# JuliaMLTools/GraphNets.jl

Measured on AMD Instinct MI355X. Metric: edges updated/sec, GNBlock fwd, 1M-edge batch, higher is better.
Workload: dtype f32; 1 GPU; C2: one shared Erdos-Renyi graph, 100k nodes / 1M edges, batch_size=1 (BASELINE configs[1]); dims=(10, 5, 0)=>(3, 4, 5), edges_whole_job=1000000, edges_per_gpu=1000000, nodes_per_gpu=100000, graphs_per_gpu=1, parallelism=single GPU

## Files before the change

### graphnets.jl_amd/csrc/gnx_device.h

```cpp
#pragma once
#ifndef GNX_JIT
#include <hip/hip_runtime.h>
#endif

namespace gnx {

struct Tile {
  int n0, n1;
  int e0, e1;
  int g;
  int win0;
  int win1;
  int flags;
};

constexpr int kPdRowsCap = 28;

struct BlockArgs {
  int de, dn, dg;
  int oe, on, og;
  const float *We, *be, *Wn, *bn, *Wg, *bg;
  int act_e, act_n, act_g;
  const float *ef, *nf, *gf;
  float *ef_out, *nf_out, *gf_out;
// ... 13 lines not shown
  float ln_eps;
  int ln_mode;
  const float* ln_stats[3];
  int ln_inline_e;
  const int* packs;
  int n_packs;
  const float *ffe_w1, *ffe_b1, *ffe_w2, *ffe_b2, *ffe_g2, *ffe_be2;
  int ffe_act1, ffe_act2;
  void* ffe_scratch;
  const float* prev_partials;
  const float* prev_gf;
  float* prev_gf_out;
  int prev_blocks;
};

__device__ __forceinline__ float relu_f(float x) {
  float r;
  asm("v_max_f32 %0, 0, %1" : "=v"(r) : "v"(x));
  return r;
}

__device__ __forceinline__ float act_apply(float x, int act) {
  switch (act) {
    case 1: return relu_f(x);
    case 2: return tanhf(x);
    case 3: return 1.f / (1.f + expf(-x));
    case 4: return 0.5f * x * (1.f + tanhf(0.7978845608028654f * (x + 0.044715f * x * x * x)));
    default: return x;
  }
}
// ... 27 lines not shown
```

### graphnets.jl_amd/csrc/gnx_forward.hip

```cpp
#include <algorithm>
#include <cstdlib>

#include "gnx_launchers.h"
#include "gnx_step_hazard.h"

namespace gnx {

static_assert(GNX_ACT_IDENTITY == 0 && GNX_ACT_RELU == 1 && GNX_ACT_TANH == 2 && GNX_ACT_SIGMOID == 3 && GNX_ACT_GELU == 4,
              "act_apply (gnx_device.h) hard-codes the activation codes");

static int32_t check_block(const gnx_graphs* h, const gnx_block_params* p, int64_t R) {
  if (!h || !p) return fail(GNX_ERR_INVALID_ARG, "NULL handle or params");
  if (R <= 0) return fail(GNX_ERR_INVALID_ARG, "n_replicas must be >= 1");
  if (R > 1 && h->G != 1)
    return fail(GNX_ERR_INVALID_ARG, "n_replicas > 1 needs a single-graph handle (shared adjacency, batch.jl:66)");
  if (R > 65535) return fail(GNX_ERR_TOO_LARGE, "n_replicas exceeds the grid limit (65535)");
  const int d[6] = {p->de, p->dn, p->dg, p->oe, p->on, p->og};
  for (int i = 0; i < 6; ++i)
    if (d[i] < 0) return fail(GNX_ERR_DIMS, "negative feature width");
  if (p->de + p->dn + p->dg == 0) return fail(GNX_ERR_DIMS, "all input widths are 0 (gnblock.jl:48, batch.jl:56)");
  if (p->oe + p->on + p->og == 0) return fail(GNX_ERR_DIMS, "all output widths are 0 (gnblock.jl:49)");
  const gnx_dense* fn[3] = {&p->edgefn, &p->nodefn, &p->graphfn};
  const int out[3] = {p->oe, p->on, p->og};
  const int in[3] = {p->de + 2 * p->dn + p->dg, p->oe + p->dn + p->dg, p->oe + p->on + p->dg};
// ... 344 lines not shown

static StepSpans step_spans(const gnx_graphs* h, const gnx_block_params* p, int64_t R, const gnx_block_step& st, size_t elem, size_t ws_extent) {
  const void* const in[3] = {st.ef, st.nf, st.gf};
  const void* const out[3] = {st.ef_out, st.nf_out, st.gf_out};
  const long long rows[3] = {(long long)h->E, (long long)h->N, (long long)h->G};
  const int in_w[3] = {p->de, p->dn, p->dg}, out_w[3] = {p->oe, p->on, p->og};
  return step_spans_of(in, out, st.workspace, st.workspace_bytes, rows, in_w, out_w, R, elem, ws_extent);
}

static bool steps_overlap_applies(const gnx_graphs* h, const gnx_block_params* p, int64_t R, uint32_t flags, hipStream_t s) {
  if (!h || !p || matrix_core_widths(*p) || (flags & GNX_FLAG_FORCE_GENERIC) || form(GNX_FLAG_NO_FORK) || profile_enabled()) return false;
  if (check_block(h, p, R) != GNX_OK) return false;
  return block_narrow_takes(h, block_probe(h, p), s);
}

static int32_t steps_schedule(const gnx_graphs* h, const gnx_block_params* p, int32_t elem, const gnx_block_step* steps, int64_t n_steps, int64_t R,
                              uint32_t flags, void* stream, bool overlap) {
  const AuxHold hold = overlap ? take_aux(h, true) : AuxHold{};
  const gnx_graphs::AuxSet* aux = hold.set;
  hipStream_t str[2] = {(hipStream_t)stream, aux ? aux->stream : nullptr};
  gnx_pending_update pend[2]{};
  auto flush = [&](int k) -> int32_t {
    if (!pend[k].workspace) return GNX_OK;
    const int32_t rc = graph_update(h, p, elem, pend[k], R, flags, str[k]);
    pend[k] = gnx_pending_update{};
    return rc;
  };
  auto run = [&](const gnx_block_step& st, int k, gnx_pending_update* next) -> int32_t {
    const gnx_pending_update* prev = pend[k].workspace ? &pend[k] : nullptr;
    return chained_step(BlockCall{h, p, elem, st.ef, st.nf, st.gf, R, st.ef_out, st.nf_out, st.gf_out, st.workspace, st.workspace_bytes, flags, str[k], GNX_PHASE_ALL},
                        prev, next);
  };
  const bool bf16 = elem == GNX_ELEM_BF16;
  const bool valid = h && p && check_block(h, p, R) == GNX_OK;
  const size_t elem_bytes = bf16 ? 2 : sizeof(float);
  const size_t ws_extent = !valid ? 0 : bf16 ? typed_ws(h, p, R, true).total : block_ws(h, p, R).total;
  if (!aux) {
    StepSpans prev;
    for (int64_t i = 0; i < n_steps; ++i) {
      const gnx_block_step& st = steps[i];
      const StepSpans cur = valid ? step_spans(h, p, R, st, elem_bytes, ws_extent) : StepSpans{};
      if (pend[0].workspace && (pend[0].workspace == st.workspace || (p && p->og > 0 && pend[0].gf_out == st.gf_out) || steps_conflict(cur, prev))) {
        if (int32_t rc = flush(0)) return rc;
      }
      prev = cur;
      gnx_pending_update next{};
      if (int32_t rc = run(st, 0, &next)) {
        (void)flush(0);
        return rc;
      }
      pend[0] = next;
    }
    return flush(0);
  }
  GNX_HIP(hipEventRecord(aux->fork, str[0]));
  GNX_HIP(hipStreamWaitEvent(str[1], aux->fork, 0));
  StepSpans recent[3];
  int32_t rc = GNX_OK;
  for (int64_t i = 0; i < n_steps && rc == GNX_OK; ++i) {
    const gnx_block_step& st = steps[i];
    const int k = (int)(i & 1), o = k ^ 1;
    const StepSpans cur = step_spans(h, p, R, st, elem_bytes, ws_extent);
    const StepOrder ord = step_order(cur, recent, i);
    if (ord.flush_own && (rc = flush(k))) break;
    if (i >= 3) {
      const hipError_t e = hipStreamWaitEvent(str[k], aux->step[(i - 3) & 3], 0);
      if (e != hipSuccess) { rc = hip_fail(e, "gnx_block_forward_steps: ordering a step behind the step three before it"); break; }
    }
    if (ord.after_other) {
      if ((rc = flush(o))) break;
      hipEvent_t ev = o == 1 ? aux->join : aux->fork;
      hipError_t e = hipEventRecord(ev, str[o]);
      if (e == hipSuccess) e = hipStreamWaitEvent(str[k], ev, 0);
      if (e != hipSuccess) { rc = hip_fail(e, "gnx_block_forward_steps: ordering a step behind the other stream"); break; }
    }
    gnx_pending_update next{};
    rc = run(st, k, &next);
    if (rc != GNX_OK) break;
    pend[k] = next;
    if (const hipError_t e = hipEventRecord(aux->step[i & 3], str[k]); e != hipSuccess) { rc = hip_fail(e, "gnx_block_forward_steps: step event"); break; }
    recent[2] = recent[1]; recent[1] = recent[0]; recent[0] = cur;
  }
  const int32_t rf0 = flush(0), rf1 = flush(1);
  const hipError_t e1 = hipEventRecord(aux->join, str[1]);
  const hipError_t e2 = hipStreamWaitEvent(str[0], aux->join, 0);
  if (rc) return rc;
  if (rf0) return rf0;
  if (rf1) return rf1;
  GNX_HIP(e1);
  GNX_HIP(e2);
  return GNX_OK;
}

int32_t gnx_block_forward_steps(const gnx_graphs* h, const gnx_block_params* p, const gnx_block_step* steps, int64_t n_steps, int64_t R, uint32_t flags,
                                void* stream) {
  if (n_steps < 0 || (n_steps > 0 && !steps)) return fail(GNX_ERR_INVALID_ARG, "gnx_block_forward_steps: steps is NULL / n_steps is negative");
  if (flags & GNX_FLAG_DEFER_GRAPH_UPDATE) return fail(GNX_ERR_INVALID_ARG, "gnx_block_forward_steps finishes every step's graph update itself");
  DeviceTurn turn((hipStream_t)stream, p && matrix_core_widths(*p));
  FormScope forms(flags);
  return steps_schedule(h, p, GNX_ELEM_F32, steps, n_steps, R, flags, stream, n_steps > 1 && steps_overlap_applies(h, p, R, flags, (hipStream_t)stream));
// ... 334 lines not shown
```

### graphnets.jl_amd/csrc/gnx_launchers.h

```cpp
#pragma once
#include "gnx_internal.h"

namespace gnx {

struct EdgeLaunch {
  const Tile* tiles; size_t n_tiles; const float* ef; size_t E;
  struct { const float* stats; const float* g; const float* b; bool inline_stats; float eps; int mode; } ln;
  const float* We; int ldw;
  const float* psrc;
  const float* pdst;
  size_t N; const int* src; const int* dst; int act;
  float* out; float* colsum;
  float* agg_out; size_t n_agg_rows; const int* chunk_row0;
  int64_t R; void* scratch; hipStream_t stream;
};

int32_t launch_block_generic(const BlockArgs& a, int64_t R, int tile_n_cap, hipStream_t s, int phase);
int32_t launch_layernorm2(const float* x, size_t rows, int d, const gnx_layernorm& l1, const gnx_layernorm& l2, float eps, int eps_mode, float* y1, float* y2, hipStream_t s);
int32_t launch_ffn_residual(const float* z, const float* x, size_t rows, int d, const gnx_ffn& ff, float* out, hipStream_t s);
int32_t launch_pad(const gnx_graphs* h, int kind, bool pad, const float* src, int d, int64_t R, float* dst, hipStream_t s);
int32_t launch_calibration(int n, hipStream_t s);
int xent_blocks(int64_t cols);
int32_t launch_xent_backward(const float* logits, const float* targets, int d, int64_t cols, const float* upstream, float* dl, hipStream_t s);
int32_t launch_xent(const float* logits, const float* targets, int d, int64_t cols, float* out, float* ws, hipStream_t s);
int32_t launch_collapse(const gnx_graphs* h, const float* ef, int d, int64_t R, float* out, hipStream_t s);
int32_t launch_collapse_padded(const gnx_graphs* h, const float* ef, int d, int64_t R, float* out, hipStream_t s);
int32_t launch_fn_input(const gnx_graphs* h, int kind, const float* ef, int de, const float* nf, int dn, const float* gf, int dg, int64_t R, float* out, hipStream_t s);

int32_t launch_block_narrow(const gnx_graphs* h, const BlockArgs& a, int64_t R, hipStream_t s, int phase, bool bf16 = false);
void warm_block_narrow(const gnx_graphs* h, const gnx_block_params* p, bool bf16 = false);
bool block_narrow_ready(const gnx_graphs* h, const BlockArgs& a, hipStream_t s);
bool block_narrow_ffe_applies(const gnx_graphs* h, const BlockArgs& a, int act1, int act2);
bool block_narrow_chain_applies(const gnx_graphs* h, const BlockArgs& a, bool bf16 = false);
bool block_narrow_takes(const gnx_graphs* h, const BlockArgs& a, hipStream_t s, bool bf16 = false);
int32_t launch_block_narrow_chained(const gnx_graphs* h, const BlockArgs& a, int64_t R, hipStream_t s, bool bf16);
bool narrow_bf16_aot(const gnx_graphs* h, const BlockArgs& a);
int32_t launch_fused_bf16(const gnx_graphs* h, const BlockArgs& a, int64_t R, hipStream_t s, int phase);
int32_t launch_chained_bf16(const gnx_graphs* h, const BlockArgs& a, int64_t R, hipStream_t s);
bool jit_eligible(const BlockArgs& a, int ept);
int32_t jit_get(const BlockArgs& a, int ept, hipStream_t s, hipFunction_t* block, hipFunction_t* graph, bool bf16 = false);
int32_t jit_get_core_post3(int d0, int d1, int d2, hipStream_t s, hipFunction_t* fn);

bool core_narrow_width(int d);
int32_t launch_ln1_rows(const float* x, size_t rows, int d, const gnx_layernorm& l1, float eps, int eps_mode, float* y, hipStream_t s);
bool core_post3_applies(const size_t rows[3], const int d[3], const gnx_ffn ff[3], bool deferred, hipStream_t s);
int32_t launch_core_post3(const float* const x[3], const size_t rows[3], const int d[3], const gnx_layernorm l2[3], const gnx_ffn ff[3], float eps,
                          int eps_mode, float* const out[3], hipStream_t s, const BlockArgs* blk, int n_rows, bool skip_edges = false);
int32_t launch_core_post(const float* x, size_t rows, int d, const gnx_layernorm& l2, const gnx_ffn& ff, float eps, int eps_mode, float* out, hipStream_t s);

int32_t launch_block_wide(const gnx_graphs* h, const BlockArgs& a, int64_t R, hipStream_t s, int phase);
size_t wide_workspace_bytes(const gnx_graphs* h, const gnx_block_params* p, int64_t R);
void warm_block_wide(const gnx_graphs* h, const gnx_block_params* p, bool rows_gemm);
bool block_wide_ln_applies(const gnx_graphs* h, const BlockArgs& a);
// ... 69 lines not shown
```

### graphnets.jl_amd/csrc/gnx_narrow.hip

```cpp
#include <cstdlib>

#include "gnx_launchers.h"
#include "gnx_narrow_launch.h"
#include "gnx_wave_kernel.h"

namespace gnx {

#define GNX_NARROW_DIMS(X) \
  X(10, 5, 0, 3, 4)        \
  X(3, 4, 5, 3, 4)         \
  X(10, 5, 3, 3, 4)        \
  X(0, 2, 0, 2, 2)         \
  X(2, 2, 2, 2, 2)         \
  X(4, 3, 2, 3, 4)         \
  X(8, 8, 8, 16, 8)        \
  X(10, 5, 3, 10, 5)       \
  X(10, 5, 0, 10, 5)
static bool narrow_aot_listed(const BlockArgs& a) {
#define GNX_CASE(DE, DN, DG, OE, ON) \
  if (a.de == DE && a.dn == DN && a.dg == DG && a.oe == OE && a.on == ON) return true;
  GNX_NARROW_DIMS(GNX_CASE)
#undef GNX_CASE
  return false;
}
// ... 70 lines not shown
    const int32_t rc = launch_chained_bf16(h, a, R, s);
    return rc == 1 ? fail(GNX_ERR_INVALID_ARG, "internal: chained bf16 launch for a width set without that kernel") : rc;
  }
#define GNX_CASE(DE, DN, DG, OE, ON)                                                                                               \
  if (a.de == DE && a.dn == DN && a.dg == DG && a.oe == OE && a.on == ON) {                                                         \
    if constexpr (OE + ON > 0) {                                                                                                   \
      return h->G == 1 ? launch_wave_g<DE, DN, DG, OE, ON, 2, false, true, false, true>(h, a, R, s, 1)                              \
                       : launch_wave_g<DE, DN, DG, OE, ON, 2, false, false, false, true>(h, a, R, s, 1);                            \
    }                                                                                                                              \
  }
  GNX_NARROW_DIMS(GNX_CASE)
#undef GNX_CASE
  return fail(GNX_ERR_INVALID_ARG, "internal: chained launch for a width set without that kernel");
}

bool block_narrow_ffe_applies(const gnx_graphs* h, const BlockArgs& a, int act1, int act2) {
  return ln_aot(h, a) && a.ln_g[0] && act1 <= GNX_ACT_RELU && act2 <= GNX_ACT_RELU && a.act_e <= GNX_ACT_RELU && h->max_in_degree <= h->wtile_e_cap &&
         !form(GNX_FLAG_NO_FFE);
}

enum NarrowRoute { NR_NONE, NR_AOT, NR_JIT };
static NarrowRoute narrow_route(const gnx_graphs* h, const BlockArgs& a, hipStream_t s, bool bf16 = false) {
  if (a.n_wtiles == 0 || a.E == 0 || wants_ln(a)) return NR_NONE;
  auto jit_ok = [&]() {
    const int ept = jit_ept(h);
    hipFunction_t fb, fg;
    return ept && jit_get(a, ept, s, &fb, &fg, bf16) == GNX_OK;
  };
  static const bool jit_all = getenv("GNX_JIT_ALL") != nullptr;
  if (jit_all && jit_ok()) return NR_JIT;
// ... 37 lines not shown
```

### graphnets.jl_amd/csrc/gnx_narrow_bf16.hip

```cpp
#include "gnx_launchers.h"
#include "gnx_narrow_launch.h"
#include "gnx_wave_kernel.h"

namespace gnx {

#define GNX_NARROW_DIMS_BF16(X) \
  X(10, 5, 0, 3, 4)             \
  X(3, 4, 5, 3, 4)

bool narrow_bf16_aot(const gnx_graphs* h, const BlockArgs& a) {
#define GNX_CASE(DE, DN, DG, OE, ON)                                     \
  if (a.de == DE && a.dn == DN && a.dg == DG && a.oe == OE && a.on == ON) \
    return h->wtile_e_cap == 64 || h->wtile_e_cap == 128 || (h->wtile_e_cap == 256 && (DE + DN) * 4 <= 64);
  GNX_NARROW_DIMS_BF16(GNX_CASE)
#undef GNX_CASE
  return false;
}

int32_t launch_fused_bf16(const gnx_graphs* h, const BlockArgs& a, int64_t R, hipStream_t s, int phase) {
#define GNX_CASE(DE, DN, DG, OE, ON) \
  if (a.de == DE && a.dn == DN && a.dg == DG && a.oe == OE && a.on == ON) return launch_fused<DE, DN, DG, OE, ON, true>(h, a, R, s, phase);
  GNX_NARROW_DIMS_BF16(GNX_CASE)
#undef GNX_CASE
  return 1;
}

int32_t launch_chained_bf16(const gnx_graphs* h, const BlockArgs& a, int64_t R, hipStream_t s) {
#define GNX_CASE(DE, DN, DG, OE, ON)                                                                                               \
  if (a.de == DE && a.dn == DN && a.dg == DG && a.oe == OE && a.on == ON) {                                                         \
    if constexpr (OE + ON > 0) {                                                                                                   \
      return h->G == 1 ? launch_wave_g<DE, DN, DG, OE, ON, 2, false, true, false, true, true>(h, a, R, s, 1)                        \
                       : launch_wave_g<DE, DN, DG, OE, ON, 2, false, false, false, true, true>(h, a, R, s, 1);                      \
    }                                                                                                                              \
  }
  GNX_NARROW_DIMS_BF16(GNX_CASE)
#undef GNX_CASE
  return 1;
}

}
```

### graphnets.jl_amd/csrc/gnx_narrow_launch.h

```cpp
#pragma once
#include <cstdlib>

#include "gnx_device.h"
#include "gnx_wave_kernel.h"

namespace gnx {

static int partial_rows(const gnx_graphs* h) { return (int)(h->G == 1 ? (h->n_wtiles() + 3) / 4 : h->n_wtiles()); }

static int graph_update_threads(const gnx_graphs* h) {
  return graph_update_threads_for_rows(h->G == 1 ? (h->n_wtiles() + 3) / 4 : h->max_wtiles_per_graph);
}

template <int DE, int DN, int DG, int OE, int ON, int EPT, bool LN, bool ONEG, bool FFE = false, bool CHAIN = false, bool BF16 = false>
static int32_t launch_wave_g(const gnx_graphs* h, const BlockArgs& a, int64_t R, hipStream_t s, int phase) {
  constexpr int C = OE + ON;
  const int n_rows = partial_rows(h);
  const unsigned grid = (unsigned)((a.n_wtiles + 3) / 4) + (CHAIN ? (unsigned)a.prev_blocks : 0u);
  if (phase & 1) {
    ProfScope ps("k_block_wave", s);
#ifdef GNX_WAVE_STAMPS_BUILD
    static unsigned long long* d_dbg = nullptr;
    static size_t dbg_cap = 0;
    const char* dump = getenv("GNX_WAVE_STAMPS_DUMP");
// ... 15 lines not shown
    }
#endif
  }
  if ((phase & 2) && a.og > 0) {
    if constexpr (C > 0) {
      const int threads = graph_update_threads(h);
      const size_t lds = sizeof(float) * (size_t)graph_update_lds_floats(C, a.dg, a.og, threads);
      ProfScope ps("k_graph_t", s);
      GNX_LAUNCH((k_graph_t<C, ONEG, BF16>), dim3((unsigned)a.G, (unsigned)R), dim3(threads), lds, s, a, n_rows);
      GNX_HIP(hipGetLastError());
    }
  }
  return GNX_OK;
}

template <int DE, int DN, int DG, int OE, int ON, int EPT, bool BF16 = false>
static bool launch_wave_pack(const gnx_graphs* h, const BlockArgs& a, int64_t R, hipStream_t s, int phase, int32_t* rc) {
  constexpr int C = OE + ON;
  if constexpr (EPT != 2 || C == 0) return false;
  else {
    if (h->G <= 1 || h->n_packs <= 0 || !a.packs || phase != 3 || a.og <= 0 || form(GNX_FLAG_NO_PACK)) return false;
    ProfScope ps("k_block_wave", s);
    GNX_LAUNCH((k_block_wave<DE, DN, DG, OE, ON, EPT, false, false, true, false, false, BF16>), dim3((unsigned)h->n_packs, (unsigned)R), dim3(kPackThreads), 0, s, a, 0);
    const hipError_t e = hipGetLastError();
    *rc = e == hipSuccess ? GNX_OK : hip_fail(e, "k_block_wave<PACK>");
    return true;
  }
}

template <int DE, int DN, int DG, int OE, int ON, int EPT, bool LN = false, bool BF16 = false>
// ... 21 lines not shown
```

### graphnets.jl_amd/csrc/gnx_step_hazard.h

```cpp
#pragma once
#include <cstddef>
#include <cstdint>

namespace gnx {

struct ByteSpan {
  uintptr_t lo = 0, hi = 0;
};

inline ByteSpan byte_span(const void* p, size_t bytes) {
  ByteSpan s;
  if (p && bytes) { s.lo = reinterpret_cast<uintptr_t>(p); s.hi = s.lo + bytes; }
  return s;
}

inline bool spans_overlap(ByteSpan a, ByteSpan b) { return a.lo < a.hi && b.lo < b.hi && a.lo < b.hi && b.lo < a.hi; }

struct StepSpans {
  ByteSpan rd[3];
  ByteSpan wr[4];
};

inline StepSpans step_spans_of(const void* const in[3], const void* const out[3], const void* ws, size_t ws_bytes, const long long rows[3],
                               const int in_w[3], const int out_w[3], long long R, size_t elem, size_t ws_extent) {
// ... 16 lines not shown
    for (const ByteSpan& r : x.rd) if (spans_overlap(w, r)) return true;
  return false;
}

struct StepOrder {
  bool flush_own = false;
  bool after_other = false;
};
inline StepOrder step_order(const StepSpans& cur, const StepSpans* recent, long long i) {
  StepOrder o;
  o.flush_own = i >= 2 && steps_conflict(cur, recent[1]);
  o.after_other = (i >= 1 && steps_conflict(cur, recent[0])) || (i >= 3 && steps_conflict(cur, recent[2]));
  return o;
}

}
```

### graphnets.jl_amd/csrc/gnx_wave_kernel.h

```cpp
#pragma once
#include "gnx_device.h"

namespace gnx {

namespace {

constexpr int kThreads = 256;

struct __attribute__((packed, aligned(4))) F4u { float x, y, z, w; };
struct __attribute__((packed, aligned(4))) F3u { float x, y, z; };
struct __attribute__((packed, aligned(4))) F2u { float x, y; };

typedef const float __attribute__((address_space(4))) * cfloatp;
__device__ __forceinline__ cfloatp as_const(const float* p) { return reinterpret_cast<cfloatp>(reinterpret_cast<size_t>(p)); }

template <int D>
__device__ __forceinline__ void load_row(const float* __restrict__ p, float (&x)[D > 0 ? D : 1]) {
  constexpr int Q = D / 4, R = D % 4;
#pragma unroll
  for (int q = 0; q < Q; ++q) {
    const F4u v = *reinterpret_cast<const F4u*>(p + 4 * q);
    x[4 * q] = v.x; x[4 * q + 1] = v.y; x[4 * q + 2] = v.z; x[4 * q + 3] = v.w;
  }
  if constexpr (R == 3) {
// ... 619 lines not shown
#define GNX_WSTAMP(i) do { } while (0)
#endif
constexpr int kPackThreads = 512;
typedef const BlockArgs __attribute__((address_space(4))) * cargsp;
template <bool FRESH>
__device__ __forceinline__ auto phase_args(const BlockArgs& a) {
  if constexpr (FRESH) {
    cargsp p = (cargsp)__builtin_amdgcn_kernarg_segment_ptr();
    asm volatile("" : "+s"(p));
    return p;
  } else {
    return &a;
  }
}

template <int DE, int DN, int DG, int OE, int ON, int EPT, bool LN, bool ONEG, bool PACK, bool FFE, bool CHAIN, bool BF16 = false>
__device__ __forceinline__ void block_wave_body(BlockArgs& a, int n_rows) {
  static_assert(!(PACK && ONEG), "packs are for batches of several graphs");
  static_assert(!BF16 || (!FFE && !LN), "bf16 features: the plain block forward and its chained form");
  static_assert(!CHAIN || (!PACK && !FFE && !LN && OE + ON > 0), "CHAIN: the two-launch form of a plain block");
  static_assert(!FFE || (LN && DE == OE && DE > 0 && EPT == 2 && (DE + DN) * OE > 96 && ((DE + DN) * OE) % 2 == 0 && GNX_WAVE_PK && !PACK),
                "FFE: a core's block (dims => dims) with LayerNorm on load, two edges per lane, streamed weights");
  constexpr int OE1 = OE > 0 ? OE : 1, ON1 = ON > 0 ? ON : 1, DE1 = DE > 0 ? DE : 1, DN1 = DN > 0 ? DN : 1, DG1 = DG > 0 ? DG : 1;
  constexpr int TEW = 64 * EPT;
  constexpr int C = OE + ON, C1 = C > 0 ? C : 1;
  constexpr int WAVES = (PACK ? kPackThreads : kThreads) / 64;
  constexpr int WSL = wave_slice_floats(OE, EPT);
  constexpr bool FRESH = FFE || (CHAIN && BF16 && !ONEG);
  __shared__ __attribute__((aligned(16))) float s_mem[WAVES * WSL];

  const int lane = threadIdx.x & 63;
  const int wv = __builtin_amdgcn_readfirstlane(threadIdx.x >> 6);
// ... 46 lines not shown
  float* s_out = s_mem + wv * WSL;
  float* s_pd = s_out + (TEW * OE + 4);
  unsigned char* s_dst = reinterpret_cast<unsigned char*>(s_pd + (64 * OE + 4));

  const cintp tw = reinterpret_cast<cintp>(reinterpret_cast<size_t>(A0->wtiles)) + (size_t)wt * (sizeof(Tile) / sizeof(int));
  const int n0 = tw[0], n1 = tw[1], e0 = tw[2], e1 = tw[3], g = tw[4];
  if constexpr (PACK) {
    tile_g = g; tile_cnt = tw[7];
    const cintp pk = reinterpret_cast<cintp>(reinterpret_cast<size_t>(A0->packs)) + (size_t)xcd_tile(bx, gx) * WAVES;
    const int wprev = wv > 0 ? pk[wv > 0 ? wv - 1 : 0] : -1;
    owner = wprev < 0 || (reinterpret_cast<cintp>(reinterpret_cast<size_t>(A0->wtiles)) + (size_t)wprev * (sizeof(Tile) / sizeof(int)))[4] != g;
  }
  const int nn = n1 - n0, ne = e1 - e0;
  GNX_WSTAMP(1);

  const size_t r = blockIdx.y;
  const auto* __restrict__ ef = DE > 0 ? feat<BF16>(A0->ef) + r * (size_t)A0->E * DE : nullptr;
  const auto* __restrict__ nf = DN > 0 ? feat<BF16>(A0->nf) + r * (size_t)A0->N * DN : nullptr;
  const cfloatp gf = DG > 0 && !BF16 ? as_const(A0->gf + (r * (size_t)A0->G + g) * DG) : nullptr;

  const bool is_node = lane < nn;
  const int nl = lane < nn ? lane : nn - 1;
  const int cp0 = A0->colptr[n0 + nl], cp1 = A0->colptr[n0 + nl + 1];
  float xn[1][DN1];
  if constexpr (DN > 0) load_row<DN>(nf + (size_t)(n0 + nl) * DN, xn[0]);
  const int cn0 = ne < TEW ? ne : TEW;
  float x[EPT][DE1];
  float xs[EPT][DN1];
  int src[EPT];
#pragma unroll
  for (int i = 0; i < EPT; ++i) {
    int ec = lane + 64 * i;
    ec = ec < cn0 ? ec : cn0 - 1;
    int e = e0 + (ec > 0 ? ec : 0);
    e = e < A0->E ? e : A0->E - 1;
    if constexpr (DE > 0) load_row<DE>(ef + (size_t)e * DE, x[i]);
    if constexpr (DN > 0) src[i] = A0->rowval[e];
  }
  if constexpr (DN > 0) {
#pragma unroll
    for (int i = 0; i < EPT; ++i) load_row<DN>(nf + (size_t)src[i] * DN, xs[i]);
  }
  float gfr[1][DG1];
  if constexpr (BF16) {
    if constexpr (DG > 0) load_row<DG>(feat<true>(A0->gf) + (r * (size_t)A0->G + g) * DG, gfr[0]);
  } else {
#pragma unroll
    for (int k = 0; k < DG; ++k) gfr[0][k] = gf[k];
  }
  if constexpr (LN) {
    ln_row<DN>(xn[0], A0->ln_g[1], A0->ln_b[1], A0->ln_eps, A0->ln_mode);
    ln_row<DG>(gfr[0], A0->ln_g[2], A0->ln_b[2], A0->ln_eps, A0->ln_mode);
  }
  GNX_WSTAMP(2);
  const auto A1 = phase_args<FRESH>(a);
  const cfloatp We = as_const(A1->We);
  const cfloatp be = as_const(A1->be ? A1->be : k_zero_bias);
  if (is_node) {
    if (nn > 1)
      for (int e = cp0 - e0; e < cp1 - e0; ++e) s_dst[e] = (unsigned char)lane;
    if constexpr (OE > 0) {
      float b[1][OE1];
#pragma unroll
      for (int j = 0; j < OE; ++j) b[0][j] = be[j];
      fma_rows<DG, OE, 1, DG1>(We + (DE + 2 * DN) * OE, gfr, b);
      fma_rows<DN, OE, 1, DN1>(We + (DE + DN) * OE, xn, b);
#pragma unroll
      for (int j = 0; j < OE; ++j) s_pd[lane * OE + j] = b[0][j];
    }
  }
  __builtin_amdgcn_wave_barrier();
  GNX_WSTAMP(3);
// ... 87 lines not shown
        fma_rows<DE, OE, EPT, DE1>(We, x, acc);
        fma_rows<DN, OE, EPT, DN1>(We + DE * OE, xs, acc);
      }
#pragma unroll
      for (int i = 0; i < EPT; ++i) {
        const int el = lane + 64 * i;
        if constexpr (FFE) {
          if (A1->act_e == 1) {
#pragma unroll
            for (int j = 0; j < OE; ++j) acc[i][j] = relu_f(acc[i][j]);
          }
        } else {
          act_row<OE1>(acc[i], A1->act_e);
        }
        if (valid[i]) {
          if constexpr (!FFE) store_row<OE>(feat<BF16>(A1->ef_out) + (r * (size_t)A1->E + e0 + c0 + el) * OE, acc[i]);
          if (nn > 1 || FFE) {
#pragma unroll
            for (int j = 0; j < OE; ++j) s_out[el * OE + j] = acc[i][j];
          }
          if (nn == 1) {
#pragma unroll
            for (int j = 0; j < OE; ++j) psum[j] += acc[i][j];
          }
        }
      }
      if constexpr (FFE) {
#pragma unroll
        for (int m = 0; m < EPT; ++m) ffv[m] = valid[m];
        ff_row0 = r * (size_t)A1->E + e0 + c0 + lane;
      }
// ... 4 lines not shown
        const int el = lane + 64 * i;
        if (el < cn) {
          const int dl = nn > 1 ? (int)s_dst[el] : 0;
          float acc[OE1];
#pragma unroll
          for (int j = 0; j < OE; ++j) acc[j] = s_pd[dl * OE + j];
#pragma unroll
          for (int k = 0; k < DE; ++k)
#pragma unroll
            for (int j = 0; j < OE; ++j) acc[j] = fmaf(We[k * OE + j], x[i][k], acc[j]);
#pragma unroll
          for (int k = 0; k < DN; ++k)
#pragma unroll
            for (int j = 0; j < OE; ++j) acc[j] = fmaf(We[(DE + k) * OE + j], xs[i][k], acc[j]);
          act_row<OE1>(acc, A1->act_e);
          store_row<OE>(feat<BF16>(A1->ef_out) + (r * (size_t)A1->E + e0 + c0 + el) * OE, acc);
          if (nn > 1) {
#pragma unroll
            for (int j = 0; j < OE; ++j) s_out[el * OE + j] = acc[j];
          } else {
#pragma unroll
            for (int j = 0; j < OE; ++j) psum[j] += acc[j];
          }
        }
      }
    }
    if constexpr (FFE) break;
  }
  __builtin_amdgcn_wave_barrier();
  GNX_WSTAMP(4);
  const auto A2 = phase_args<FRESH>(a);
  const cfloatp Wn = as_const(A2->Wn);
  const cfloatp bn = as_const(A2->bn ? A2->bn : k_zero_bias);

  float v[C1];
#pragma unroll
  for (int c = 0; c < C1; ++c) v[c] = 0.f;
  if constexpr (OE > 0) {
    if (nn == 1) {
#pragma unroll
      for (int j = 0; j < OE; ++j) {
        const float tot = wave_sum(psum[j]);
        v[j] = lane == 0 ? tot : 0.f;
      }
    } else if (is_node) {
      for (int e = cp0 - e0; e < cp1 - e0; ++e) {
#pragma unroll
        for (int j = 0; j < OE; ++j) v[j] += s_out[e * OE + j];
// ... 3 lines not shown
  if constexpr (ON > 0) {
    if (is_node) {
      float acc1[1][ON1];
      float (&acc)[ON1] = acc1[0];
#pragma unroll
      for (int j = 0; j < ON; ++j) acc[j] = bn[j];
      fma_rows<DG, ON, 1, DG1>(Wn + (OE + DN) * ON, gfr, acc1);
      float vin[1][OE1];
#pragma unroll
      for (int k = 0; k < OE; ++k) vin[0][k] = v[k];
      fma_rows<OE, ON, 1, OE1>(Wn, vin, acc1);
      fma_rows<DN, ON, 1, DN1>(Wn + OE * ON, xn, acc1);
      act_row<ON1>(acc, A2->act_n);
#pragma unroll
      for (int j = 0; j < ON; ++j) v[OE + j] = acc[j];
      store_row<ON>(feat<BF16>(A2->nf_out) + (r * (size_t)A2->N + n0 + lane) * ON, acc);
    }
  }

  if (A2->og > 0) {
    if constexpr (C > 0) {
      float sel[(C + 15) / 16];
#pragma unroll
      for (int g = 0; g < (C + 15) / 16; ++g) sel[g] = 0.f;
#pragma unroll
      for (int c = 0; c < C; ++c) {
        const float s16 = row16_sum(v[c]);
        sel[c >> 4] = (lane & 15) == (c & 15) ? s16 : sel[c >> 4];
      }
      float tot = 0.f;
#pragma unroll
// ... 7 lines not shown
    }
  }
  GNX_WSTAMP(5);
  } while (0);
#ifdef GNX_WAVE_STAMPS_BUILD
  if (active && g_wave_dbg && lane == 0 && blockIdx.y == 0) {
    wst_[6] = clock64();
    unsigned long long* o = g_wave_dbg + (size_t)wt * 8;
    for (int i = 0; i < 7; ++i) o[i] = wst_[i];
    o[7] = ((unsigned long long)__builtin_amdgcn_s_getreg((31 << 11) | 20) << 32) | __builtin_amdgcn_s_getreg((31 << 11) | 4);
  }
#endif
  const auto A3 = phase_args<FRESH>(a);
  if (A3->og > 0) {
    if constexpr (C > 0) {
      const size_t r = blockIdx.y;
      constexpr int CP = (C + 3) / 4 * 4;
      float* __restrict__ pbase = A3->partials + r * (size_t)n_rows * CP;
      if constexpr (PACK) {
        __shared__ float s_rows[WAVES][C1];
        if (lane < C) s_rows[wv][lane] = active ? mine : 0.f;
        GraphWaveRegs gr;
        if (active && owner) graph_wave_prefetch<C>(a, lane, gr);
        __syncthreads();
        if (active && owner) {
          float rr[8];
#pragma unroll
          for (int k = 0; k < 8; ++k) rr[k] = (k < tile_cnt && wv + k < WAVES && lane < C) ? 0.f + s_rows[(wv + k) < WAVES ? wv + k : 0][lane < C ? lane : 0] : 0.f;
          const float xs = ((rr[0] + rr[1]) + (rr[2] + rr[3])) + ((rr[4] + rr[5]) + (rr[6] + rr[7]));
          graph_update_wave<C, BF16>(a, xs, tile_g, r, lane, s_mem + wv * WSL, gr);
        }
      } else if constexpr (ONEG) {
        __shared__ float s_blk[WAVES][C1];
// ... 54 lines not shown
    }
  }
}

template <int DE, int DN, int DG, int OE, int ON, int EPT, bool LN = false, bool ONEG = false, bool PACK = false, bool FFE = false, bool CHAIN = false,
          bool BF16 = false>
__global__ __launch_bounds__(PACK ? kPackThreads : kThreads) __attribute__((amdgpu_num_sgpr(GNX_WAVE_SGPRS))) void k_block_wave(BlockArgs a, int n_rows) {
  static_assert(!FFE, "the FFE form is k_block_wave_ffe");
  block_wave_body<DE, DN, DG, OE, ON, EPT, LN, ONEG, PACK, false, CHAIN, BF16>(a, n_rows);
}
template <int DE, int DN, int DG, int OE, int ON, int EPT, bool ONEG>
__global__ __launch_bounds__(kThreads) __attribute__((amdgpu_waves_per_eu(4))) void k_block_wave_ffe(BlockArgs a, int n_rows) {
  block_wave_body<DE, DN, DG, OE, ON, EPT, true, ONEG, false, true, false>(a, n_rows);
}

template <int C, bool ONEG = false, bool BF16 = false>
__global__ void k_graph_t(BlockArgs a, int n_rows) {
  extern __shared__ float s_g[];
  constexpr int CP = (C + 3) / 4 * 4;
  const int g = blockIdx.x;
  const int t0 = ONEG ? 0 : a.wtile_off[g], t1 = ONEG ? (a.n_wtiles + 3) / 4 : a.wtile_off[g + 1];
  const float* base = a.partials + blockIdx.y * (size_t)n_rows * CP;
  if (blockDim.x == 64) graph_update_rows<C, true, 16, BF16>(a, a.gf, a.gf_out, base, g, blockIdx.y, t0, t1, (int)threadIdx.x, 64, s_g);
  else graph_update_rows<C, false, 16, BF16>(a, a.gf, a.gf_out, base, g, blockIdx.y, t0, t1, (int)threadIdx.x, (int)blockDim.x, s_g);
}

}
```

Baseline: 54.16 billion edges/s.

## Batch independent forward steps into one multi-slot kernel launch

Groups up to eight consecutive non-conflicting block-forward steps into a single launch. Each step's input and output pointers go into a table placed after BlockArgs in the kernel arguments, and grid.y selects the step's slot. This is meant to cut per-step launch and event overhead and let several steps fill the GPU together. In exchange it adds more hazard-grouping logic and larger kernel arguments, and it only applies to single-replica narrow width sets.

```diff
diff --git a/graphnets.jl_amd/csrc/gnx_device.h b/graphnets.jl_amd/csrc/gnx_device.h
--- a/graphnets.jl_amd/csrc/gnx_device.h
+++ b/graphnets.jl_amd/csrc/gnx_device.h
@@ -51,6 +51,17 @@
   int prev_blocks;
 };
 
+struct RunSlot {
+  const float *ef, *nf, *gf;
+  float *ef_out, *nf_out, *gf_out;
+  float* partials;
+};
+constexpr int kRunSlots = 8;
+struct RunTable {
+  RunSlot slot[kRunSlots];
+};
+constexpr unsigned kRunTableOffset = (unsigned)((sizeof(BlockArgs) + 7) / 8 * 8);
+
 __device__ __forceinline__ float relu_f(float x) {
   float r;
   asm("v_max_f32 %0, 0, %1" : "=v"(r) : "v"(x));
diff --git a/graphnets.jl_amd/csrc/gnx_forward.hip b/graphnets.jl_amd/csrc/gnx_forward.hip
--- a/graphnets.jl_amd/csrc/gnx_forward.hip
+++ b/graphnets.jl_amd/csrc/gnx_forward.hip
@@ -382,10 +382,22 @@
   return block_narrow_takes(h, block_probe(h, p), s);
 }
 
+constexpr int kStepsRunDefault = 8;
+static_assert(kRunMax == kRunSlots, "gnx_step_hazard.h groups what gnx_device.h's table holds");
+static int steps_run_max() {
+  static const int v = [] {
+    const char* e = getenv("GNX_STEPS_RUN_MAX");
+    const int n = e && *e ? atoi(e) : kStepsRunDefault;
+    return n < 1 ? 1 : (n > kRunMax ? kRunMax : n);
+  }();
+  return v;
+}
+
 static int32_t steps_schedule(const gnx_graphs* h, const gnx_block_params* p, int32_t elem, const gnx_block_step* steps, int64_t n_steps, int64_t R,
                               uint32_t flags, void* stream, bool overlap) {
   const AuxHold hold = overlap ? take_aux(h, true) : AuxHold{};
   const gnx_graphs::AuxSet* aux = hold.set;
+  const bool two = aux != nullptr;
   hipStream_t str[2] = {(hipStream_t)stream, aux ? aux->stream : nullptr};
   gnx_pending_update pend[2]{};
   auto flush = [&](int k) -> int32_t {
@@ -403,36 +415,52 @@
   const bool valid = h && p && check_block(h, p, R) == GNX_OK;
   const size_t elem_bytes = bf16 ? 2 : sizeof(float);
   const size_t ws_extent = !valid ? 0 : bf16 ? typed_ws(h, p, R, true).total : block_ws(h, p, R).total;
-  if (!aux) {
-    StepSpans prev;
-    for (int64_t i = 0; i < n_steps; ++i) {
-      const gnx_block_step& st = steps[i];
-      const StepSpans cur = valid ? step_spans(h, p, R, st, elem_bytes, ws_extent) : StepSpans{};
-      if (pend[0].workspace && (pend[0].workspace == st.workspace || (p && p->og > 0 && pend[0].gf_out == st.gf_out) || steps_conflict(cur, prev))) {
-        if (int32_t rc = flush(0)) return rc;
+  bool can_fuse = valid && R == 1 && !(flags & GNX_FLAG_FORCE_GENERIC) && steps_run_max() > 1 && !profile_enabled();
+  auto slot_of = [&](const gnx_block_step& st, RunSlot& sl, BlockArgs* run_args) -> bool {
+    Prepared q(BlockCall{h, p, elem, st.ef, st.nf, st.gf, R, st.ef_out, st.nf_out, st.gf_out, st.workspace, st.workspace_bytes, flags, str[0], GNX_PHASE_ALL});
+    if (q.rc) return false;
+    if (run_args) {
+      if (!block_narrow_run_applies(h, q.a, bf16)) return can_fuse = false;
+      *run_args = q.a;
+    }
+    sl = RunSlot{q.a.ef, q.a.nf, q.a.gf, q.a.ef_out, q.a.nf_out, q.a.gf_out, q.a.partials};
+    return true;
+  };
+  if (two) {
+    GNX_HIP(hipEventRecord(aux->fork, str[0]));
+    GNX_HIP(hipStreamWaitEvent(str[1], aux->fork, 0));
+  }
+  RunSpans recent[3];
+  int32_t rc = GNX_OK;
+  int64_t i = 0;
+  for (int64_t j = 0; i < n_steps && rc == GNX_OK; ++j) {
+    const gnx_block_step& st = steps[i];
+    RunSpans cur;
+    RunTable tab{};
+    BlockArgs run_args{};
+    cur.step[0] = valid ? step_spans(h, p, R, st, elem_bytes, ws_extent) : StepSpans{};
+    cur.n = 1;
+    if (can_fuse && n_steps - i >= 2) {
+      RunSpans win = cur;
+      while (i + win.n < n_steps) {
+        const StepSpans sp = step_spans(h, p, R, steps[i + win.n], elem_bytes, ws_extent);
+        if (!run_takes(win, sp, steps_run_max())) break;
+        win.step[win.n++] = sp;
       }
-      prev = cur;
-      gnx_pending_update next{};
-      if (int32_t rc = run(st, 0, &next)) {
-        (void)flush(0);
-        return rc;
-      }
-      pend[0] = next;
-    }
-    return flush(0);
-  }
-  GNX_HIP(hipEventRecord(aux->fork, str[0]));
-  GNX_HIP(hipStreamWaitEvent(str[1], aux->fork, 0));
-  StepSpans recent[3];
-  int32_t rc = GNX_OK;
-  for (int64_t i = 0; i < n_steps && rc == GNX_OK; ++i) {
-    const gnx_block_step& st = steps[i];
-    const int k = (int)(i & 1), o = k ^ 1;
-    const StepSpans cur = step_spans(h, p, R, st, elem_bytes, ws_extent);
-    const StepOrder ord = step_order(cur, recent, i);
-    if (ord.flush_own && (rc = flush(k))) break;
-    if (i >= 3) {
-      const hipError_t e = hipStreamWaitEvent(str[k], aux->step[(i - 3) & 3], 0);
+      bool ok = window_is_run(win.n, i, n_steps, steps_run_max());
+      for (int z = 0; ok && z < win.n; ++z) ok = slot_of(steps[i + z], tab.slot[z], z == 0 ? &run_args : nullptr);
+      if (ok) cur = win;
+    }
+    const int k = two ? (int)(j & 1) : 0, o = k ^ 1;
+    StepOrder ord;
+    if (two) {
+      ord = run_order(cur, recent, j);
+    } else {
+      ord.flush_own = pend[0].workspace && (pend[0].workspace == st.workspace || (p && p->og > 0 && pend[0].gf_out == st.gf_out) || runs_conflict(cur, recent[0]));
+    }
+    if ((ord.flush_own || cur.n > 1) && (rc = flush(k))) break;
+    if (two && j >= 3) {
+      const hipError_t e = hipStreamWaitEvent(str[k], aux->step[(j - 3) & 3], 0);
       if (e != hipSuccess) { rc = hip_fail(e, "gnx_block_forward_steps: ordering a step behind the step three before it"); break; }
     }
     if (ord.after_other) {
@@ -442,16 +470,26 @@
       if (e == hipSuccess) e = hipStreamWaitEvent(str[k], ev, 0);
       if (e != hipSuccess) { rc = hip_fail(e, "gnx_block_forward_steps: ordering a step behind the other stream"); break; }
     }
-    gnx_pending_update next{};
-    rc = run(st, k, &next);
+    if (cur.n > 1) {
+      rc = launch_block_narrow_run(h, run_args, tab, cur.n, str[k], bf16);
+    } else {
+      gnx_pending_update next{};
+      rc = run(st, k, &next);
+      if (rc == GNX_OK) pend[k] = next;
+    }
     if (rc != GNX_OK) break;
-    pend[k] = next;
-    if (const hipError_t e = hipEventRecord(aux->step[i & 3], str[k]); e != hipSuccess) { rc = hip_fail(e, "gnx_block_forward_steps: step event"); break; }
+    if (two) {
+      if (const hipError_t e = hipEventRecord(aux->step[j & 3], str[k]); e != hipSuccess) { rc = hip_fail(e, "gnx_block_forward_steps: step event"); break; }
+    }
     recent[2] = recent[1]; recent[1] = recent[0]; recent[0] = cur;
-  }
-  const int32_t rf0 = flush(0), rf1 = flush(1);
-  const hipError_t e1 = hipEventRecord(aux->join, str[1]);
-  const hipError_t e2 = hipStreamWaitEvent(str[0], aux->join, 0);
+    i += cur.n;
+  }
+  const int32_t rf0 = flush(0), rf1 = two ? flush(1) : GNX_OK;
+  hipError_t e1 = hipSuccess, e2 = hipSuccess;
+  if (two) {
+    e1 = hipEventRecord(aux->join, str[1]);
+    e2 = hipStreamWaitEvent(str[0], aux->join, 0);
+  }
   if (rc) return rc;
   if (rf0) return rf0;
   if (rf1) return rf1;
diff --git a/graphnets.jl_amd/csrc/gnx_launchers.h b/graphnets.jl_amd/csrc/gnx_launchers.h
--- a/graphnets.jl_amd/csrc/gnx_launchers.h
+++ b/graphnets.jl_amd/csrc/gnx_launchers.h
@@ -37,6 +37,10 @@
 bool narrow_bf16_aot(const gnx_graphs* h, const BlockArgs& a);
 int32_t launch_fused_bf16(const gnx_graphs* h, const BlockArgs& a, int64_t R, hipStream_t s, int phase);
 int32_t launch_chained_bf16(const gnx_graphs* h, const BlockArgs& a, int64_t R, hipStream_t s);
+bool block_narrow_run_applies(const gnx_graphs* h, const BlockArgs& a, bool bf16);
+bool narrow_bf16_run(const gnx_graphs* h, const BlockArgs& a);
+int32_t launch_block_narrow_run(const gnx_graphs* h, const BlockArgs& a, const RunTable& t, int Z, hipStream_t s, bool bf16);
+int32_t launch_run_bf16(const gnx_graphs* h, const BlockArgs& a, const RunTable& t, int Z, hipStream_t s);
 bool jit_eligible(const BlockArgs& a, int ept);
 int32_t jit_get(const BlockArgs& a, int ept, hipStream_t s, hipFunction_t* block, hipFunction_t* graph, bool bf16 = false);
 int32_t jit_get_core_post3(int d0, int d1, int d2, hipStream_t s, hipFunction_t* fn);
diff --git a/graphnets.jl_amd/csrc/gnx_narrow.hip b/graphnets.jl_amd/csrc/gnx_narrow.hip
--- a/graphnets.jl_amd/csrc/gnx_narrow.hip
+++ b/graphnets.jl_amd/csrc/gnx_narrow.hip
@@ -108,6 +108,38 @@
   return fail(GNX_ERR_INVALID_ARG, "internal: chained launch for a width set without that kernel");
 }
 
+#define GNX_NARROW_RUN_DIMS(X) \
+  X(10, 5, 0, 3, 4)            \
+  X(3, 4, 5, 3, 4)             \
+  X(10, 5, 3, 3, 4)            \
+  X(0, 2, 0, 2, 2)             \
+  X(2, 2, 2, 2, 2)             \
+  X(4, 3, 2, 3, 4)
+bool block_narrow_run_applies(const gnx_graphs* h, const BlockArgs& a, bool bf16) {
+  if (!block_narrow_chain_applies(h, a, bf16)) return false;
+  if (bf16) return narrow_bf16_run(h, a);
+#define GNX_CASE(DE, DN, DG, OE, ON) \
+  if (a.de == DE && a.dn == DN && a.dg == DG && a.oe == OE && a.on == ON) return true;
+  GNX_NARROW_RUN_DIMS(GNX_CASE)
+#undef GNX_CASE
+  return false;
+}
+int32_t launch_block_narrow_run(const gnx_graphs* h, const BlockArgs& a, const RunTable& t, int Z, hipStream_t s, bool bf16) {
+  if (bf16) {
+    const int32_t rc = launch_run_bf16(h, a, t, Z, s);
+    return rc == 1 ? fail(GNX_ERR_INVALID_ARG, "internal: bf16 run launch for a width set without that kernel") : rc;
+  }
+#define GNX_CASE(DE, DN, DG, OE, ON)                                                                                               \
+  if (a.de == DE && a.dn == DN && a.dg == DG && a.oe == OE && a.on == ON) {                                                         \
+    if constexpr (OE + ON > 0) {                                                                                                   \
+      return h->G == 1 ? launch_wave_run<DE, DN, DG, OE, ON, true>(h, a, t, Z, s) : launch_wave_run<DE, DN, DG, OE, ON, false>(h, a, t, Z, s); \
+    }                                                                                                                              \
+  }
+  GNX_NARROW_RUN_DIMS(GNX_CASE)
+#undef GNX_CASE
+  return fail(GNX_ERR_INVALID_ARG, "internal: run launch for a width set without that kernel");
+}
+
 bool block_narrow_ffe_applies(const gnx_graphs* h, const BlockArgs& a, int act1, int act2) {
   return ln_aot(h, a) && a.ln_g[0] && act1 <= GNX_ACT_RELU && act2 <= GNX_ACT_RELU && a.act_e <= GNX_ACT_RELU && h->max_in_degree <= h->wtile_e_cap &&
          !form(GNX_FLAG_NO_FFE);
diff --git a/graphnets.jl_amd/csrc/gnx_narrow_bf16.hip b/graphnets.jl_amd/csrc/gnx_narrow_bf16.hip
--- a/graphnets.jl_amd/csrc/gnx_narrow_bf16.hip
+++ b/graphnets.jl_amd/csrc/gnx_narrow_bf16.hip
@@ -38,4 +38,25 @@
   return 1;
 }
 
+#define GNX_NARROW_RUN_DIMS_BF16(X) \
+  X(10, 5, 0, 3, 4, false)          \
+  X(3, 4, 5, 3, 4, true)
+bool narrow_bf16_run(const gnx_graphs* h, const BlockArgs& a) {
+#define GNX_CASE(DE, DN, DG, OE, ON, SEVERAL) \
+  if (a.de == DE && a.dn == DN && a.dg == DG && a.oe == OE && a.on == ON) return h->G == 1 || SEVERAL;
+  GNX_NARROW_RUN_DIMS_BF16(GNX_CASE)
+#undef GNX_CASE
+  return false;
 }
+int32_t launch_run_bf16(const gnx_graphs* h, const BlockArgs& a, const RunTable& t, int Z, hipStream_t s) {
+#define GNX_CASE(DE, DN, DG, OE, ON, SEVERAL)                                                                \
+  if (a.de == DE && a.dn == DN && a.dg == DG && a.oe == OE && a.on == ON) {                                   \
+    if (h->G == 1) return launch_wave_run<DE, DN, DG, OE, ON, true, true>(h, a, t, Z, s);                     \
+    if constexpr (SEVERAL) return launch_wave_run<DE, DN, DG, OE, ON, false, true>(h, a, t, Z, s);            \
+  }
+  GNX_NARROW_RUN_DIMS_BF16(GNX_CASE)
+#undef GNX_CASE
+  return 1;
+}
+
+}
diff --git a/graphnets.jl_amd/csrc/gnx_narrow_launch.h b/graphnets.jl_amd/csrc/gnx_narrow_launch.h
--- a/graphnets.jl_amd/csrc/gnx_narrow_launch.h
+++ b/graphnets.jl_amd/csrc/gnx_narrow_launch.h
@@ -53,6 +53,26 @@
   return GNX_OK;
 }
 
+template <int DE, int DN, int DG, int OE, int ON, bool ONEG, bool BF16 = false>
+static int32_t launch_wave_run(const gnx_graphs* h, const BlockArgs& a, const RunTable& t, int Z, hipStream_t s) {
+  constexpr int C = OE + ON;
+  if (Z < 1 || Z > kRunSlots) return fail(GNX_ERR_INVALID_ARG, "internal: a run of more steps than the table has slots");
+  const int n_rows = partial_rows(h);
+  {
+    ProfScope ps("k_block_wave", s);
+    GNX_LAUNCH((k_block_wave_run<DE, DN, DG, OE, ON, 2, ONEG, BF16>), dim3((unsigned)((a.n_wtiles + 3) / 4), (unsigned)Z), dim3(kThreads), 0, s, a, t, n_rows);
+    GNX_HIP(hipGetLastError());
+  }
+  if (a.og > 0) {
+    const int threads = graph_update_threads(h);
+    const size_t lds = sizeof(float) * (size_t)graph_update_lds_floats(C, a.dg, a.og, threads);
+    ProfScope ps("k_graph_t", s);
+    GNX_LAUNCH((k_graph_run<C, ONEG, BF16>), dim3((unsigned)a.G, (unsigned)Z), dim3(threads), lds, s, a, t, n_rows);
+    GNX_HIP(hipGetLastError());
+  }
+  return GNX_OK;
+}
+
 template <int DE, int DN, int DG, int OE, int ON, int EPT, bool BF16 = false>
 static bool launch_wave_pack(const gnx_graphs* h, const BlockArgs& a, int64_t R, hipStream_t s, int phase, int32_t* rc) {
   constexpr int C = OE + ON;
diff --git a/graphnets.jl_amd/csrc/gnx_step_hazard.h b/graphnets.jl_amd/csrc/gnx_step_hazard.h
--- a/graphnets.jl_amd/csrc/gnx_step_hazard.h
+++ b/graphnets.jl_amd/csrc/gnx_step_hazard.h
@@ -54,4 +54,48 @@
   return o;
 }
 
+constexpr int kRunMax = 8;
+constexpr int kRunTailMin = 4;
+
+struct RunSpans {
+  int n = 0;
+  StepSpans step[kRunMax];
+};
+
+inline bool run_conflicts_step(const RunSpans& r, const StepSpans& s) {
+  for (int a = 0; a < r.n; ++a)
+    if (steps_conflict(r.step[a], s)) return true;
+  return false;
 }
+
+inline bool runs_conflict(const RunSpans& x, const RunSpans& y) {
+  for (int b = 0; b < y.n; ++b)
+    if (run_conflicts_step(x, y.step[b])) return true;
+  return false;
+}
+
+inline bool run_takes(const RunSpans& run, const StepSpans& next, int run_max) {
+  return run.n >= 1 && run.n < run_max && run.n < kRunMax && !run_conflicts_step(run, next);
+}
+
+inline bool window_is_run(int n, long long first, long long n_steps, int run_max) {
+  return n >= 2 && (n == run_max || (first + n == n_steps && n >= kRunTailMin));
+}
+
+inline RunSpans group_run(const StepSpans* spans, long long n_steps, long long first, int run_max) {
+  RunSpans run;
+  if (first >= n_steps) return run;
+  run.step[run.n++] = spans[first];
+  while (first + run.n < n_steps && run_takes(run, spans[first + run.n], run_max)) { run.step[run.n] = spans[first + run.n]; ++run.n; }
+  if (!window_is_run(run.n, first, n_steps, run_max)) run.n = 1;
+  return run;
+}
+
+inline StepOrder run_order(const RunSpans& cur, const RunSpans* recent, long long j) {
+  StepOrder o;
+  o.flush_own = j >= 2 && runs_conflict(cur, recent[1]);
+  o.after_other = (j >= 1 && runs_conflict(cur, recent[0])) || (j >= 3 && runs_conflict(cur, recent[2]));
+  return o;
+}
+
+}
diff --git a/graphnets.jl_amd/csrc/gnx_wave_kernel.h b/graphnets.jl_amd/csrc/gnx_wave_kernel.h
--- a/graphnets.jl_amd/csrc/gnx_wave_kernel.h
+++ b/graphnets.jl_amd/csrc/gnx_wave_kernel.h
@@ -657,8 +657,17 @@
   }
 }
 
-template <int DE, int DN, int DG, int OE, int ON, int EPT, bool LN, bool ONEG, bool PACK, bool FFE, bool CHAIN, bool BF16 = false>
+typedef const RunSlot __attribute__((address_space(4))) * cslotp;
+__device__ __forceinline__ cslotp run_slot() {
+  typedef const char __attribute__((address_space(4))) * ccharp;
+  cslotp p = (cslotp)((ccharp)__builtin_amdgcn_kernarg_segment_ptr() + kRunTableOffset) + blockIdx.y;
+  asm volatile("" : "+s"(p));
+  return p;
+}
+
+template <int DE, int DN, int DG, int OE, int ON, int EPT, bool LN, bool ONEG, bool PACK, bool FFE, bool CHAIN, bool BF16 = false, bool RUN = false>
 __device__ __forceinline__ void block_wave_body(BlockArgs& a, int n_rows) {
+  static_assert(!RUN || (!PACK && !FFE && !LN && !CHAIN && OE + ON > 0), "RUN: the two-launch form of a plain block, one slot per step");
   static_assert(!(PACK && ONEG), "packs are for batches of several graphs");
   static_assert(!BF16 || (!FFE && !LN), "bf16 features: the plain block forward and its chained form");
   static_assert(!CHAIN || (!PACK && !FFE && !LN && OE + ON > 0), "CHAIN: the two-launch form of a plain block");
@@ -735,10 +744,17 @@
   const int nn = n1 - n0, ne = e1 - e0;
   GNX_WSTAMP(1);
 
-  const size_t r = blockIdx.y;
-  const auto* __restrict__ ef = DE > 0 ? feat<BF16>(A0->ef) + r * (size_t)A0->E * DE : nullptr;
-  const auto* __restrict__ nf = DN > 0 ? feat<BF16>(A0->nf) + r * (size_t)A0->N * DN : nullptr;
-  const cfloatp gf = DG > 0 && !BF16 ? as_const(A0->gf + (r * (size_t)A0->G + g) * DG) : nullptr;
+  const size_t r = RUN ? 0 : blockIdx.y;
+  const float *ef_in = nullptr, *nf_in = nullptr, *gf_in = nullptr;
+  if constexpr (RUN) {
+    const cslotp S0 = run_slot();
+    ef_in = S0->ef; nf_in = S0->nf; gf_in = S0->gf;
+  } else {
+    ef_in = A0->ef; nf_in = A0->nf; gf_in = A0->gf;
+  }
+  const auto* __restrict__ ef = DE > 0 ? feat<BF16>(ef_in) + r * (size_t)A0->E * DE : nullptr;
+  const auto* __restrict__ nf = DN > 0 ? feat<BF16>(nf_in) + r * (size_t)A0->N * DN : nullptr;
+  const cfloatp gf = DG > 0 && !BF16 ? as_const(gf_in + (r * (size_t)A0->G + g) * DG) : nullptr;
 
   const bool is_node = lane < nn;
   const int nl = lane < nn ? lane : nn - 1;
@@ -764,7 +780,7 @@
   }
   float gfr[1][DG1];
   if constexpr (BF16) {
-    if constexpr (DG > 0) load_row<DG>(feat<true>(A0->gf) + (r * (size_t)A0->G + g) * DG, gfr[0]);
+    if constexpr (DG > 0) load_row<DG>(feat<true>(gf_in) + (r * (size_t)A0->G + g) * DG, gfr[0]);
   } else {
 #pragma unroll
     for (int k = 0; k < DG; ++k) gfr[0][k] = gf[k];
@@ -777,6 +793,8 @@
   const auto A1 = phase_args<FRESH>(a);
   const cfloatp We = as_const(A1->We);
   const cfloatp be = as_const(A1->be ? A1->be : k_zero_bias);
+  [[maybe_unused]] float* run_ef_out = nullptr;
+  if constexpr (RUN) run_ef_out = run_slot()->ef_out;
   if (is_node) {
     if (nn > 1)
       for (int e = cp0 - e0; e < cp1 - e0; ++e) s_dst[e] = (unsigned char)lane;
@@ -894,7 +912,7 @@
           act_row<OE1>(acc[i], A1->act_e);
         }
         if (valid[i]) {
-          if constexpr (!FFE) store_row<OE>(feat<BF16>(A1->ef_out) + (r * (size_t)A1->E + e0 + c0 + el) * OE, acc[i]);
+          if constexpr (!FFE) store_row<OE>(feat<BF16>(RUN ? run_ef_out : A1->ef_out) + (r * (size_t)A1->E + e0 + c0 + el) * OE, acc[i]);
           if (nn > 1 || FFE) {
 #pragma unroll
             for (int j = 0; j < OE; ++j) s_out[el * OE + j] = acc[i][j];
@@ -929,7 +947,7 @@
 #pragma unroll
             for (int j = 0; j < OE; ++j) acc[j] = fmaf(We[(DE + k) * OE + j], xs[i][k], acc[j]);
           act_row<OE1>(acc, A1->act_e);
-          store_row<OE>(feat<BF16>(A1->ef_out) + (r * (size_t)A1->E + e0 + c0 + el) * OE, acc);
+          store_row<OE>(feat<BF16>(RUN ? run_ef_out : A1->ef_out) + (r * (size_t)A1->E + e0 + c0 + el) * OE, acc);
           if (nn > 1) {
 #pragma unroll
             for (int j = 0; j < OE; ++j) s_out[el * OE + j] = acc[j];
@@ -947,6 +965,8 @@
   const auto A2 = phase_args<FRESH>(a);
   const cfloatp Wn = as_const(A2->Wn);
   const cfloatp bn = as_const(A2->bn ? A2->bn : k_zero_bias);
+  [[maybe_unused]] float* run_nf_out = nullptr;
+  if constexpr (RUN) run_nf_out = run_slot()->nf_out;
 
   float v[C1];
 #pragma unroll
@@ -980,7 +1000,7 @@
       act_row<ON1>(acc, A2->act_n);
 #pragma unroll
       for (int j = 0; j < ON; ++j) v[OE + j] = acc[j];
-      store_row<ON>(feat<BF16>(A2->nf_out) + (r * (size_t)A2->N + n0 + lane) * ON, acc);
+      store_row<ON>(feat<BF16>(RUN ? run_nf_out : A2->nf_out) + (r * (size_t)A2->N + n0 + lane) * ON, acc);
     }
   }
 
@@ -1018,9 +1038,11 @@
   const auto A3 = phase_args<FRESH>(a);
   if (A3->og > 0) {
     if constexpr (C > 0) {
-      const size_t r = blockIdx.y;
+      const size_t r = RUN ? 0 : blockIdx.y;
       constexpr int CP = (C + 3) / 4 * 4;
-      float* __restrict__ pbase = A3->partials + r * (size_t)n_rows * CP;
+      float* part;
+      if constexpr (RUN) part = run_slot()->partials; else part = A3->partials;
+      float* __restrict__ pbase = part + r * (size_t)n_rows * CP;
       if constexpr (PACK) {
         __shared__ float s_rows[WAVES][C1];
         if (lane < C) s_rows[wv][lane] = active ? mine : 0.f;
@@ -1105,6 +1127,11 @@
   block_wave_body<DE, DN, DG, OE, ON, EPT, true, ONEG, false, true, false>(a, n_rows);
 }
 
+template <int DE, int DN, int DG, int OE, int ON, int EPT, bool ONEG, bool BF16 = false>
+__global__ __launch_bounds__(kThreads) __attribute__((amdgpu_num_sgpr(GNX_WAVE_SGPRS))) void k_block_wave_run(BlockArgs a, RunTable t, int n_rows) {
+  block_wave_body<DE, DN, DG, OE, ON, EPT, false, ONEG, false, false, false, BF16, true>(a, n_rows);
+}
+
 template <int C, bool ONEG = false, bool BF16 = false>
 __global__ void k_graph_t(BlockArgs a, int n_rows) {
   extern __shared__ float s_g[];
@@ -1116,4 +1143,17 @@
   else graph_update_rows<C, false, 16, BF16>(a, a.gf, a.gf_out, base, g, blockIdx.y, t0, t1, (int)threadIdx.x, (int)blockDim.x, s_g);
 }
 
-}
+template <int C, bool ONEG = false, bool BF16 = false>
+__global__ void k_graph_run(BlockArgs a, RunTable t, int n_rows) {
+  extern __shared__ float s_g[];
+  const int g = blockIdx.x;
+  const int t0 = ONEG ? 0 : a.wtile_off[g], t1 = ONEG ? (a.n_wtiles + 3) / 4 : a.wtile_off[g + 1];
+  const cslotp S = run_slot();
+  const float* const base = S->partials;
+  const float* const gf = S->gf;
+  float* const gf_out = S->gf_out;
+  if (blockDim.x == 64) graph_update_rows<C, true, 16, BF16>(a, gf, gf_out, base, g, 0, t0, t1, (int)threadIdx.x, 64, s_g);
+  else graph_update_rows<C, false, 16, BF16>(a, gf, gf_out, base, g, 0, t0, t1, (int)threadIdx.x, (int)blockDim.x, s_g);
+}
+
+}
```

Result: faster. 58.20 billion edges/s (median of 6 runs) (+7.4%).
